# Fleming-Sung/mpc-limX-control

Measured on AMD Instinct MI355X. Metric: QP solves/sec, 13-state N=10 SRBM MPC, batch=65536 at 1/2/4/8 MI355X, higher is better.
Workload: dtype f64; 1 GPU; TRON1 SRBM MPC 13x6 N=10 (box, R = 1e-05 I), linearise+discretise+condense+solve + min-cost selection, global batch 65536 split over 1 GPU(s); global_batch=65536, batch_per_gpu=65536, horizon=10, nx=13, nu=6, config=B, parallelism=dp1, selection=record fused into the solve kernels (last workgroup) (single GPU), max_solver_iters=7, select=fused, kernel=k_mpc_pair, lib_build_id=cfb06c8e6fa2

## Files before the change

include/mpcqp.h:

```cpp
#ifndef MPCQP_H
#define MPCQP_H

#include <stddef.h>
#include <stdint.h>

#ifdef __cplusplus
extern "C" {
#endif

#define MPCQP_OK 0
#define MPCQP_ERR_BAD_DIMS 1
#define MPCQP_ERR_INFEASIBLE 2
#define MPCQP_ERR_ITER_LIMIT 3
#define MPCQP_ERR_NOT_PD 4
#define MPCQP_ERR_DEVICE 5
#define MPCQP_ERR_BAD_ARG 6
#define MPCQP_ERR_NO_DEVICE 7

#define MPCQP_INFTY 1e20

#define MPCQP_MAX_NX 32
#define MPCQP_MAX_NU 16
#define MPCQP_MAX_N 32
#define MPCQP_MAX_NV 256
// ... 132 lines not shown
                    const double *eeVel, const unsigned char *contact, const double *quat,
                    const double *acc);

int mpcqp_enable_timing(mpcqp_ctx *ctx, int on);
double mpcqp_last_kernel_ms(mpcqp_ctx *ctx, int which);
double mpcqp_kernel_ms_sum(mpcqp_ctx *ctx, int which, int *count);

int mpcqp_count_solver_flops(mpcqp_ctx *ctx, int on);
double mpcqp_solver_flops(mpcqp_ctx *ctx, int *launches);

int mpcqp_ctx_pair_dedup(const mpcqp_ctx *ctx);
int mpcqp_ctx_pair_w4_min(const mpcqp_ctx *ctx);
int mpcqp_count_covered(mpcqp_ctx *ctx, int on);
long long mpcqp_covered(mpcqp_ctx *ctx, int *launches);

int mpcqp_debug_phase_cycles(mpcqp_ctx *ctx, uint64_t *out, int n);

const char *mpcqp_status_string(int status);
const char *mpcqp_build_id(void);
int mpcqp_device_count(void);

#ifdef __cplusplus
}
#endif
#endif
```

mpc-limx-control_amd/csrc/fast_kernels.hpp:

```cpp
#pragma once
#include <hip/hip_runtime.h>

#include "../../include/mpcqp.h"

#ifdef MPCQP_VARIANT_TAG
extern "C" const char *mpcqp_variant_tag_fn(void) { return MPCQP_VARIANT_TAG; }
#endif

#ifndef MPCQP_W32
#define MPCQP_W32 3
#endif
#ifndef MPCQP_W64
#define MPCQP_W64 2
#endif
#include "condense.hpp"
#include "fused.hpp"
#include "mpc_fused.hpp"

namespace mpcqp {

struct FastKernels {
    const void *mpc_gen = nullptr;
    const void *pair = nullptr, *pair_gen = nullptr;
    const void *pair_w4 = nullptr, *pair_gen_w4 = nullptr;
    int pair_w4_min = 0;
    int pair_can_dedup = 0;
    int pair_dedup = 0;
    size_t pair_lds = 0;
    const void *wg = nullptr;
    size_t wg_lds = 0;
    int wg_threads = 0;
    const void *dense = nullptr;
    size_t dense_lds = 0;
    int dense_threads = 0;
    const void *disc = nullptr, *cs = nullptr, *mpc = nullptr;
    const void *mpc_list = nullptr;
    size_t disc_lds = 0, cs_lds = 0, mpc_lds = 0;
    int nx = 0, nu = 0;
    int prim_nf = 0;
    int nf = 0;
    int crash_k = 0, crash_p = 0;
    int crash_k_wg = 0, crash_p_wg = 0;
// ... 94 lines not shown
```

mpc-limx-control_amd/csrc/fast_pair.hip:

```cpp
#include <hip/hip_runtime.h>

#include "../../include/mpcqp.h"
#include "fast_kernels.hpp"
#include "mpc_pair.hpp"

namespace mpcqp {
namespace {

template <int NU, int N, int MODEL, bool GEN, int W>
__global__ void __launch_bounds__(64, W) k_mpc_pair(MpcArgs a) {
    extern __shared__ __attribute__((aligned(16))) unsigned char smem_p[];
    pair_mpc<NU, N, MODEL, GEN, W>(a, smem_p);
}

template <int NU, int N, int MODEL>
void add_pair(FastKernels &k) {
    k.pair = (const void *)&k_mpc_pair<NU, N, MODEL, false, 3>;
    k.pair_w4 = (const void *)&k_mpc_pair<NU, N, MODEL, false, 4>;
    if constexpr (MODEL == 0) {
        k.pair_gen = (const void *)&k_mpc_pair<NU, N, MODEL, true, 3>;
        k.pair_gen_w4 = (const void *)&k_mpc_pair<NU, N, MODEL, true, 4>;
    }
    k.pair_lds = PairLayout<NU, N, MODEL>::lds_bytes;
#ifdef MPCQP_INPUT_ALIAS
    k.pair_can_dedup = 0;
#else
    k.pair_can_dedup = (MPCQP_PAIR_SORT && MODEL == 0 && 2 * N <= 32) ? 1 : 0;
#endif
    k.crash_k = MPCQP_PAIR_CRASH ? kPairCrashK : 0;
    k.crash_p = MPCQP_PAIR_CRASH ? kPairCrashP : 0;
}

}

bool add_fast_pair(int model, int N, bool fric, int nfmax, FastKernels &k) {
    static_assert(kPairNF == kPairCap, "one capacity");
    (void)nfmax;
    if (fric || N != 10) return false;
    if (model == MPCQP_MODEL_SRBM && k.nu == 6) { add_pair<6, 10, 0>(k); return true; }
    if (model == MPCQP_MODEL_LITERAL && k.nu == 3) { add_pair<3, 10, 1>(k); return true; }
    return false;
}

// ... 2 lines not shown
```

mpc-limx-control_amd/csrc/mpc_fused.hpp:

```cpp
#pragma once
#include "condense.hpp"
#include "gi_reg.hpp"
#include "gi_solver.hpp"

namespace mpcqp {

#ifndef MPCQP_REG_TILES
#define MPCQP_REG_TILES 1
#endif
template <int NF>
constexpr bool kRegTiles = MPCQP_REG_TILES && NF > 32;

struct MpcArgs {
    int B;
    double Ts, mass;
    double Ibinv[9];
    const double *qd, *pd;
    const double *qm, *pm;
    const double *fq, *fp;
    const double *rmat;
    double fz_min, fz_max, fxy_max, u_min, u_max, mu;
    int max_iter, max_free;
    int crash_p;
    int crash_p_wg;
    double blo_v, blo_t, bhi_v, bhi_t, tlo_v, tlo_t, thi_v, thi_t;
    const double *lin, *x0, *xref;
    const uint64_t *contact;
    double *U, *cost;
    int *status, *iters;
    unsigned long long *stamps;
    double *flops_acc;
    int dedup;
    unsigned long long *cov_acc;
    int cut;
    const double *state;
    const double *feet;
    const double *cmd;
    const double *phase;
    int cands;
    float swing, stance;
    int *ovf;
    int ovf_cap;
    unsigned long long *warm;
    int warm_words;
    unsigned long long *sel;
    long long sel_base;
    long long *sel_rec;
    int sel_final;
// ... 91 lines not shown
    __threadfence();
    sel_final_reduce(a, nV, scratch, tid, kSelNone);
}
__device__ __forceinline__ void sel_commit(const MpcArgs &a, unsigned long long k, int nV,
                                           bool wrote, unsigned long long *scratch, int groups = -1,
                                           bool fresh = false) {
    sel_commit_t(a, k, nV, wrote, scratch, groups, (int)threadIdx.x, fresh);
}

constexpr int kListSubs = 64, kListStride = 32;
constexpr int kListHeadWords = kListSubs * kListStride;
__host__ __device__ constexpr int ovf_list_cap(long long B) {
    return (int)((B + kListSubs - 1) / kListSubs) + 2;
}
__device__ __forceinline__ void wg_list_append(int *list, int cap, int b0, bool d0, int b1,
                                               bool d1) {
    const int n = (d0 ? 1 : 0) + (d1 ? 1 : 0);
    if (!n) return;
    const int s = (int)(blockIdx.x % kListSubs);
    const int i = __hip_atomic_fetch_add(&list[s * kListStride], n, __ATOMIC_RELAXED,
                                         __HIP_MEMORY_SCOPE_AGENT);
    int *ids = list + kListHeadWords + s * cap + i;
    if (d0) *ids++ = b0;
    if (d1) *ids = b1;
}
struct OvfView {
    int *list;
    int cap, cnt, incl, total;
    __device__ __forceinline__ int id(int i) const {
        const int s = __popcll(__ballot(incl <= i));
        const int excl = __shfl(incl - cnt, s, kWave);
        return list[kListHeadWords + s * cap + (i - excl)];
    }
};
// ... 294 lines not shown
    C.L.rowfix = D + Lay::oMisc;
    C.L.ys = D + Lay::oMisc;
    int *ip = reinterpret_cast<int *>(D + Lay::nDoubles);
    C.L.fid = ip;
    C.L.pos = ip + NF;
    C.L.st = reinterpret_cast<unsigned char *>(ip + NF + NV);
    C.L.cb = D + Lay::oCB;

    double lin[8];
    mpc_load_inputs<Lay, NU, N, GEN>(a, b, D, lin);
    MPCQP_CUT(a.cut, 11);
    gi_setup(C);
    if (C.nf > a.max_free || (listed && C.nf > NF)) C.status = ST_BAD_DIMS;
    wave_sync();
    if (!listed && a.ovf && C.nf > NF && C.nf <= a.max_free) {
        if (ln == 0) wg_list_append(a.ovf, a.ovf_cap, b, true, 0, false);
        return;
    }
    mpc_model_terms<Lay, NU, MODEL>(a, D, lin);
    MPCQP_CUT(a.cut, 13);
    MPCQP_STAMP(a.stamps, 0, tst);
    MPCQP_CUT(a.cut, 1);

    mpc_condensed_terms<Lay, NU, N, MODEL>(a, D);
    MPCQP_STAMP(a.stamps, 1, tst);
    MPCQP_CUT(a.cut, 2);

    const int nf = C.nf;
    const bool ok = C.status == ST_OK && nf > 0;
    double gp = 0.0;
    if (ok && ln < nf) {
// ... 87 lines not shown
```

mpc-limx-control_amd/csrc/mpc_pair.hpp:

```cpp
#pragma once
#include "half_ops.hpp"
#include "mpc_fused.hpp"

namespace mpcqp {

template <int W>
constexpr int pair_pf() {
#ifdef MPCQP_PF_DUAL
    return MPCQP_PF_DUAL;
#else
    return W >= 4 ? 4 : 8;
#endif
}
#ifndef MPCQP_PAIR_SORT
#define MPCQP_PAIR_SORT 1
#endif
#ifndef MPCQP_CHOL_CB
#define MPCQP_CHOL_CB 2
#endif
#ifndef MPCQP_CHOL_PF
#define MPCQP_CHOL_PF 4
#endif
#ifndef MPCQP_PAIR_FOLD
#define MPCQP_PAIR_FOLD 1
// ... 96 lines not shown
    const uint64_t right = half_ballot(hl < N && ph < sw);
    const uint64_t left = half_ballot(hl < N && !(ph < sw));
    return spread_even(left) | (spread_even(right) << 1);
}

__device__ __forceinline__ int row_bcast_u32(int v, int j) {
    switch (j) {
#define MPCQP_RB(i) case i: return __builtin_amdgcn_mov_dpp(v, 0x150 + i, 0xf, 0xf, false);
        MPCQP_RB(0) MPCQP_RB(1) MPCQP_RB(2) MPCQP_RB(3) MPCQP_RB(4) MPCQP_RB(5) MPCQP_RB(6)
        MPCQP_RB(7) MPCQP_RB(8) MPCQP_RB(9) MPCQP_RB(10) MPCQP_RB(11) MPCQP_RB(12) MPCQP_RB(13)
        MPCQP_RB(14) MPCQP_RB(15)
#undef MPCQP_RB
        default: return 0;
    }
}
template <bool GEN, int N>
__device__ __forceinline__ int pair_sorted_instance(const MpcArgs &a, unsigned &same,
                                                    unsigned &cand) {
    const int ln = lane(), c = ln & 15;
    int g0, wq;
    if constexpr (!GEN && 2 * N <= 32) {
        const int w = (int)blockIdx.x, ngf = a.B >> 4;
        if (w < 8 * ngf) {
            wq = w / ngf;
            g0 = 16 * (w - wq * ngf);
        } else {
            wq = w - 8 * ngf;
            g0 = 16 * ngf;
        }
    } else {
        const int wv = xcd_order((int)blockIdx.x, (int)gridDim.x);
        g0 = (2 * wv) & ~15;
        wq = wv & 7;
    }
    const int gn = a.B - g0 < 16 ? a.B - g0 : 16;
    int rank = 0;
    [[maybe_unused]] unsigned eq = 0, xw = 0;
    if constexpr (!GEN && 2 * N <= 32) {
        unsigned key = ~0u;
        if (c < gn) key = (unsigned)a.contact[g0 + c];
        if (a.dedup && c < gn) {
            const long long xb = __double_as_longlong(a.x0[(size_t)(g0 + c) * 13 + 3]);
            xw = (unsigned)xb ^ (unsigned)(xb >> 32);
        }
        unsigned lt = 0;
#pragma unroll
        for (int j = 0; j < 16; ++j) {
            const unsigned kj = (unsigned)row_bcast_u32((int)key, j);
            lt |= (j < gn && kj < key) ? (1u << j) : 0u;
            eq |= (j < gn && kj == key) ? (1u << j) : 0u;
        }
        const unsigned below = (1u << c) - 1u;
        const bool first = (eq & below) == 0u;
        const unsigned lead = (unsigned)(__ballot(ln < 16 && c < gn && first) & 0xffffull);
        rank = first ? __popc(lead & lt)
                     : __popc(lead) + __popc(lt & ~lead) + __popc(eq & below) - 1;
    } else {
        unsigned long long key = ~0ull;
// ... 114 lines not shown
    static_assert(!GEN || MODEL == 0, "generated inputs are defined for the SRBM model");
    static_assert(MODEL == 0 || MODEL == 1, "TRON1 models only");
    using Lay = PairLayout<NU, N, MODEL>;
    using Sup = XSupport<MODEL>;
    constexpr int NX = 13, NS = NX + NU, NF = kPairNF, NV = Lay::NV, SD = Lay::SD, NP = kHalf;
#ifdef MPCQP_INPUT_ALIAS
    constexpr bool kDedup = false;
#else
    constexpr bool kDedup = MPCQP_PAIR_SORT && MODEL == 0 && !GEN && 2 * N <= 32;
#endif
    MPCQP_STAMP_INIT(tst);
    const int ln = lane(), hl = ln & (kHalf - 1);
    const bool up = ln >= kHalf;
    int bq = 2 * xcd_order((int)blockIdx.x, (int)gridDim.x) + (up ? 1 : 0);
    unsigned same = 0, cand = 0;
    if constexpr (MPCQP_PAIR_SORT && MODEL == 0) bq = pair_sorted_instance<GEN, N>(a, same, cand);
    bool valid = bq < a.B;
    unsigned cov = 0;
    const int b = valid ? bq : a.B - 1;
    [[maybe_unused]] const int b_ = b;
    unsigned char *Dbase = smem + (up ? Lay::bytes : 0);
    double *D = reinterpret_cast<double *>(Dbase);
    signed char *fid = reinterpret_cast<signed char *>(Dbase + Lay::oFid);
    signed char *pos = reinterpret_cast<signed char *>(Dbase + Lay::oPos);
    double *X0 = D + Lay::oX0, *X1 = D + Lay::oX1, *Ax = D + Lay::oAx, *A2x = D + Lay::oA2x;
    double *xr = D + Lay::oXr, *x0g = D + Lay::oX0v, *UV = D + Lay::oUV;
    double *S = D + Lay::oS;
    const double *Rm = a.rmat;
    const double *Qd = a.qd, *Pd = a.pd;

    double lin[8];
// ... 74 lines not shown
#pragma unroll
                    for (int c = 0; c < NC; ++c)
                        if (half_ballot(d[c] != 0ull) == 0u) cov |= bit[c];
                };
                do {
                    const unsigned tw = (unsigned)__builtin_amdgcn_readlane((int)todo, 0),
                                   tu = (unsigned)__builtin_amdgcn_readlane((int)todo, kHalf);
                    if (((tw & (tw - 1u)) | (tu & (tu - 1u))) == 0u) trip(PairInt<1>{});
                    else trip(PairInt<CH>{});
                } while (__ballot(todo != 0u) != 0ull);
                if (3 * __popcll(contact & kSched) > NF) cov = 0u;
            }
            if (!leads && cov) {
                valid = false;
                cov = 0u;
            }
            if (__ballot(valid) == 0ull) {
                if (a.sel)
                    sel_commit_t(a, kSelNone, NV, false,
                                 reinterpret_cast<unsigned long long *>(smem) + Lay::oR, -1, ln);
                return;
            }
        }
#pragma unroll
        for (int r = 0; r < RX; ++r)
            if (hl + r * kHalf < NXR) xr[hl + r * kHalf] = v[r];
        if (hl < NX) x0g[hl] = x0l;
    }
    wave_sync();
    MPCQP_CUT(a.cut, 11);
// ... 986 lines not shown
    MPCQP_STAMP(a.stamps, 8, tst);
    MPCQP_CUT(a.cut, 7);
    int lno = lane();
    asm volatile("" : "+v"(lno));
    const int hlo = lno & (kHalf - 1);
    double *Do = reinterpret_cast<double *>(smem + (lno >= kHalf ? Lay::bytes : 0));
    const unsigned char *Dob = smem + (lno >= kHalf ? Lay::bytes : 0);
    const signed char *fido = reinterpret_cast<const signed char *>(Dob + Lay::oFid);
    const signed char *poso = reinterpret_cast<const signed char *>(Dob + Lay::oPos);
    const uint64_t *ctlo = reinterpret_cast<const uint64_t *>(Dob + Lay::oCt);
    const int bo = (int)(long long)ctlo[1];
    const bool defer = a.ovf && nf > NF && nf <= a.max_free;
    {
        const int b0 = __builtin_amdgcn_readlane(bo, 0), b1 = __builtin_amdgcn_readlane(bo, kHalf);
        const uint64_t dm = __ballot(defer && bo >= 0);
        if (dm && lno == 0) wg_list_append(a.ovf, a.ovf_cap, b0, dm & 1ull, b1, (dm >> kHalf) & 1ull);
    }
    if constexpr (GEN) {
        if (a.warm) {
            unsigned long long *wl = reinterpret_cast<unsigned long long *>(Do + Lay::oRow);
            wave_sync();
            if (hlo < a.warm_words) wl[hlo] = 0ull;
            wave_sync();
            if (bo >= 0 && hlo < nf && nf <= NF && act2) {
                const int v = fido[hlo];
                if (act2 & 1) atomicOr(&wl[v >> 6], 1ull << (v & 63));
                if (act2 & 2) atomicOr(&wl[(NV + v) >> 6], 1ull << ((NV + v) & 63));
            }
            wave_sync();
            if (bo >= 0 && hlo < a.warm_words) a.warm[(size_t)bo * a.warm_words + hlo] = wl[hlo];
            wave_sync();
// ... 65 lines not shown
```

mpc-limx-control_amd/csrc/mpcqp_kernels.hip:

```cpp
#include <hip/hip_runtime.h>
#include <unistd.h>

#include <math.h>
#include <stdio.h>
#include <stdlib.h>
#include <string.h>

#include <algorithm>
#include <new>
#include <vector>

#include "../../include/mpcqp.h"

#include "fast_kernels.hpp"
#include "gi_solver.hpp"
#include "gi_wg.hpp"

using namespace mpcqp;

namespace {

struct CondenseArgs {
    ModelConst mc;
    int B;
// ... 367 lines not shown
    if (model == MPCQP_MODEL_SRBM && nu == 6) {
        if (N == 10) found = pick_fast_srbm10(fric, nprim, k);
        if (N == 20) found = pick_fast_srbm20(fric, nprim, k);
    }
    if (model == MPCQP_MODEL_LITERAL && nu == 3 && !fric) found = pick_fast_literal(N, nprim, k);
    if (found && pair_enabled()) add_fast_pair(model, N, fric, nprim, k);
    if (k.pair && k.crash_k > 0)
        if (const char *e = getenv("MPCQP_CRASH_P")) k.crash_p = std::max(0, atoi(e));
    if (k.pair) {
        const char *e = getenv("MPCQP_PAIR_DEDUP");
        k.pair_dedup = k.pair_can_dedup && !(e && e[0] == '0');
    }
    if (k.pair) {
        k.pair_w4_min = kPairW4Min;
        if (const char *e = getenv("MPCQP_PAIR_W4_MIN")) k.pair_w4_min = std::max(0, atoi(e));
    }
    if (k.pair)
        if (const char *e = getenv("MPCQP_PAIR_LDS_PAD")) k.pair_lds += (size_t)std::max(0, atoi(e));
    if (found) {
        k.prim_nf = k.pair ? kPairCap : k.nf;
        if (nfmax > k.prim_nf) add_fast_wg(model, N, fric, k);
    }
    if (k.crash_k_wg > 0)
        if (const char *e = getenv("MPCQP_CRASH_P_WG")) k.crash_p_wg = std::max(0, atoi(e));
    return found;
}

void inv3(const double *A, double *Ai) {
    const double a = A[0], b = A[3], c = A[6], d = A[1], e = A[4], f = A[7], g = A[2],
                 h = A[5], i = A[8];
// ... 66 lines not shown
    double *scratchH = nullptr, *scratchF = nullptr;
    size_t scratch_cap = 0;
    bool fast = false;
    FastKernels fk;
    double *dqd = nullptr, *dpd = nullptr;
    double *dFQ = nullptr, *dFP = nullptr;
    double *dAB = nullptr;
    size_t ab_cap = 0;
    unsigned long long *dstamps = nullptr;
    double *dflops = nullptr;
    bool flops_on = false;
    int flops_launches = 0;
    unsigned long long *dcov = nullptr;
    bool cov_on = false;
    int cov_launches = 0;
    unsigned long long *dsel = nullptr;
    int *dlist = nullptr;
    size_t list_cap = 0;
    int list_par = 0;
    int wg_grid = 0;
    void *hbuf = nullptr;
    size_t hbuf_cap = 0;
    void *pin = nullptr;
    size_t pin_cap = 0;
    hipStream_t hstream = nullptr;
    hipEvent_t hev = nullptr;
    hipStream_t hs_in = nullptr, hs_out = nullptr;
    hipEvent_t hev_in[8] = {}, hev_k[8] = {};
    bool hd_ok = false;
    bool hd_off = false;
// ... 372 lines not shown
                     hipMemcpy(c->dFQ, fq.data(), sizeof(double) * nx * nx, hipMemcpyHostToDevice) != hipSuccess ||
                     hipMemcpy(c->dFP, fp.data(), sizeof(double) * nx * nx, hipMemcpyHostToDevice) != hipSuccess)) {
            mpcqp_ctx_destroy(c);
            return MPCQP_ERR_DEVICE;
        }
        if (pick_fast_dense(nx, nu, m->N, toep, c->fk)) {
            c->fast = true;
            set_lds(c->fk.dense, c->fk.dense_lds);
            if (const char *e = getenv("MPCQP_CRASH_P_WG")) c->fk.crash_p_wg = std::max(0, atoi(e));
        }
    }
    if (!c->fast && nfmax > kWave) {
        mpcqp_ctx_destroy(c);
        return MPCQP_ERR_BAD_DIMS;
    }
    if (c->fast && c->fk.wg) {
        int dev_cus = 0, nb = 0;
        hipDeviceGetAttribute(&dev_cus, hipDeviceAttributeMultiprocessorCount, device);
        set_lds(c->fk.wg, c->fk.wg_lds);
        hipOccupancyMaxActiveBlocksPerMultiprocessor(&nb, c->fk.wg, c->fk.wg_threads, c->fk.wg_lds);
        c->wg_grid = std::max(1, nb) * std::max(1, dev_cus);
    }
    c->m.Q = c->m.R = c->m.P = nullptr;
    *out = c;
    return MPCQP_OK;
}

int mpcqp_ctx_fast_path(const mpcqp_ctx *c) {
    if (!c || !c->fast) return 0;
    if (c->fk.dense) return 3;
// ... 47 lines not shown
        hipStreamSynchronize(c->stream) != hipSuccess)
        return -1.0;
    for (int i = 0; i < kFlopsSlots; ++i) v += h[i * kFlopsStride];
    if (launches) *launches = c->flops_launches;
    c->flops_launches = 0;
    return v;
}

int mpcqp_ctx_pair_dedup(const mpcqp_ctx *c) {
    return c && c->fast && c->fk.pair && !c->fk.dense ? c->fk.pair_dedup : 0;
}

int mpcqp_ctx_pair_w4_min(const mpcqp_ctx *c) {
    if (!c || !c->fast || !c->fk.pair || c->fk.dense || !c->fk.pair_w4) return 0;
    return c->fk.pair_w4_min;
}

int mpcqp_count_covered(mpcqp_ctx *c, int on) {
    if (!c) return MPCQP_ERR_BAD_ARG;
    if (on && !c->dcov) {
        hipSetDevice(c->device);
        if (hipMalloc(&c->dcov, sizeof(unsigned long long) * kFlopsWords) != hipSuccess ||
            hipMemsetAsync(c->dcov, 0, sizeof(unsigned long long) * kFlopsWords, c->stream) != hipSuccess) {
            hipFree(c->dcov);
            c->dcov = nullptr;
            return MPCQP_ERR_DEVICE;
        }
    }
    c->cov_on = on != 0;
    return MPCQP_OK;
// ... 41 lines not shown
int mpcqp_ctx_destroy(mpcqp_ctx *c) {
    if (!c) return MPCQP_ERR_BAD_ARG;
    hipSetDevice(c->device);
    if (c->stream) hipStreamSynchronize(c->stream);
    hipFree(c->dQ);
    hipFree(c->dR);
    hipFree(c->dP);
    hipFree(c->dqd);
    hipFree(c->dpd);
    hipFree(c->dFQ);
    hipFree(c->dFP);
    hipFree(c->dAB);
    hipFree(c->dstamps);
    hipFree(c->dflops);
    hipFree(c->dcov);
    hipFree(c->dsel);
    hipFree(c->dlist);
    hipFree(c->hbuf);
    for (int i = 0; i < 3; ++i)
        if (c->hg_exec[i]) hipGraphExecDestroy(c->hg_exec[i]);
    if (c->pin) hipHostFree(c->pin);
    if (c->hev) hipEventDestroy(c->hev);
    if (c->hstream) hipStreamDestroy(c->hstream);
    for (int i = 0; i < 8; ++i) {
        if (c->hev_in[i]) hipEventDestroy(c->hev_in[i]);
        if (c->hev_k[i]) hipEventDestroy(c->hev_k[i]);
    }
    if (c->hs_in) hipStreamDestroy(c->hs_in);
    if (c->hs_out) hipStreamDestroy(c->hs_out);
    hipFree(c->rbuf);
// ... 11 lines not shown
}

int mpcqp_set_stream(mpcqp_ctx *c, void *stream) {
    if (!c) return MPCQP_ERR_BAD_ARG;
    if (c->own_stream && c->stream) {
        hipStreamSynchronize(c->stream);
        hipStreamDestroy(c->stream);
    }
    c->own_stream = false;
    c->stream = (hipStream_t)stream;
    return MPCQP_OK;
}

int mpcqp_sync(mpcqp_ctx *c) {
    if (!c) return MPCQP_ERR_BAD_ARG;
    return hip_status(hipStreamSynchronize(c->stream));
}

int mpcqp_enable_timing(mpcqp_ctx *c, int on) {
    if (!c) return MPCQP_ERR_BAD_ARG;
    if (on && !c->ev_ok) {
        hipSetDevice(c->device);
        hipEvent_t *evs = &c->ev[0][0][0];
        constexpr int nev = 4 * mpcqp_ctx::kTimingRing * 2;
        for (int i = 0; i < nev; ++i)
            if (hipEventCreate(&evs[i]) != hipSuccess) {
                for (int j = 0; j < i; ++j) hipEventDestroy(evs[j]);
                return MPCQP_ERR_DEVICE;
            }
        c->ev_ok = true;
    }
// ... 107 lines not shown
    {
        const bool lit = m.model == MPCQP_MODEL_LITERAL;
        a.blo_v = lit ? m.u_min : m.fz_min;
        a.blo_t = lit ? m.u_min : -m.fxy_max;
        a.bhi_v = lit ? -m.u_max : -m.fz_max;
        a.bhi_t = lit ? -m.u_max : -m.fxy_max;
        a.tlo_v = -kFeasTol * (1.0 + fabs(a.blo_v));
        a.tlo_t = -kFeasTol * (1.0 + fabs(a.blo_t));
        a.thi_v = -kFeasTol * (1.0 + fabs(a.bhi_v));
        a.thi_t = -kFeasTol * (1.0 + fabs(a.bhi_t));
    }
    a.stamps = c->dstamps;
    a.flops_acc = c->flops_on ? c->dflops : nullptr;
    a.dedup = c->fk.pair_dedup;
    a.cov_acc = c->cov_on ? c->dcov : nullptr;
    a.cut = 0;
#ifdef MPCQP_CUTS
    if (const char *e = getenv("MPCQP_CUT")) a.cut = atoi(e);
#endif
    return a;
}

static int launch(const void *k, int B, size_t lds, hipStream_t s, void *arg) {
    void *args[] = {arg};
    return hip_status(hipLaunchKernel(k, dim3(B), dim3(64), args, lds, s));
}

static int ensure_bytes(mpcqp_ctx *c, void **buf, size_t *cap, size_t bytes) {
    if (*cap >= bytes) return MPCQP_OK;
    if (*buf) hipStreamSynchronize(c->stream);
// ... 42 lines not shown
    if (c->dlist) hipStreamSynchronize(c->stream);
    hipFree(c->dlist);
    c->dlist = nullptr;
    c->list_cap = 0;
    ++c->buf_gen;
    const size_t stride = list_stride((size_t)B);
    if (hipMalloc(&c->dlist, sizeof(int) * 2 * stride) != hipSuccess ||
        hipMemsetAsync(c->dlist, 0, sizeof(int) * kListHeadWords, c->stream) != hipSuccess ||
        hipMemsetAsync(c->dlist + stride, 0, sizeof(int) * kListHeadWords, c->stream) != hipSuccess)
        return MPCQP_ERR_DEVICE;
    c->list_cap = B;
    c->list_par = 0;
    return MPCQP_OK;
}

static int launch_mpc(mpcqp_ctx *c, bool gen, int B, MpcArgs *a, bool may_overflow = true) {
    a->ovf = nullptr;
    int *list = nullptr, *rearm = nullptr;
    if (c->fk.wg && !gen && may_overflow) {
        const int rc = ensure_list(c, B);
        if (rc) return rc;
        const size_t stride = list_stride(c->list_cap);
        list = c->dlist + (c->list_par ? stride : 0);
        rearm = c->dlist + (c->list_par ? 0 : stride);
        a->ovf = list;
        a->ovf_cap = ovf_list_cap((long long)c->list_cap);
    }
    const void *pk = gen ? c->fk.pair_gen : c->fk.pair;
    if (pk && B >= c->fk.pair_w4_min && c->fk.pair_w4_min > 0) {
        const void *p4 = gen ? c->fk.pair_gen_w4 : c->fk.pair_w4;
        if (p4) pk = p4;
    }
    a->sel_final = a->ovf ? 0 : 1;
    if (a->flops_acc && pk) ++c->flops_launches;
    if (a->cov_acc && pk) ++c->cov_launches;
    tbegin(c, 2);
    int rc = pk ? launch(pk, (B + 1) / 2, c->fk.pair_lds, c->stream, a)
                : launch(gen ? c->fk.mpc_gen : c->fk.mpc, B, c->fk.mpc_lds, c->stream, a);
    tend(c, 2);
    if (rc || !a->ovf) return rc;
    a->sel_final = 1;
    void *args[] = {a, &list, &rearm};
    const int grid = std::max(1, std::min(B, c->wg_grid));
    tbegin(c, 3);
    rc = hip_status(hipLaunchKernel(c->fk.wg, dim3(grid), dim3(c->fk.wg_threads), args, c->fk.wg_lds,
                                    c->stream));
    tend(c, 3);
    c->list_par ^= 1;
    return rc;
}

int mpcqp_batch_condense(mpcqp_ctx *c, int B, const double *x0, const double *xref,
                         const double *lin, double *H, double *f) {
    if (!c || !x0 || !xref || !lin || !H || !f || B < 0) return MPCQP_ERR_BAD_ARG;
    if (B == 0) return MPCQP_OK;
    hipSetDevice(c->device);
    CondenseArgs a = batch_condense_args(c, B, x0, xref, lin, H, f);
    const size_t lds = set_lds((const void *)k_condense,
                               sizeof(double) * condense_lds_doubles(c->m.nx, c->m.nu, c->m.N));
    tbegin(c, 0);
    hipLaunchKernelGGL(k_condense, dim3(B), dim3(64), lds, c->stream, a);
    tend(c, 0);
    return hip_status(hipGetLastError());
// ... 205 lines not shown
        return rc;
    }
    int rc = mpcqp_batch_solve(c, B, x0, xref, lin, contact, U, cost, status, iters);
    if (!rc) rc = mpcqp_batch_select_record(c, B, cost, status, U, index_base, record);
    return rc;
}

int mpcqp_ctx_reserve(mpcqp_ctx *c, int B) {
    if (!c || B < 0) return MPCQP_ERR_BAD_ARG;
    if (B == 0) return MPCQP_OK;
    hipSetDevice(c->device);
    const size_t ab = (size_t)c->m.nx * (c->m.nx + c->m.nu);
    int rc = ensure_bytes(c, &c->hbuf, &c->hbuf_cap, host_stage_bytes(c, B));
    if (!rc) rc = ensure_bytes(c, &c->fkbuf, &c->fkbuf_cap, sizeof(double) * 15 * (size_t)B);
    if (!rc && c->fast && c->fk.wg) rc = ensure_list(c, B);
    if (!rc && c->fast && c->fk.mpc_gen)
        rc = ensure_bytes(c, &c->rbuf, &c->rbuf_cap, rollout_bytes(c, B, 1));
    if (!rc && c->warm_on && c->fast && c->fk.mpc_gen) rc = ensure_warm(c, B);
    if (!rc && !c->fast) rc = ensure_bytes(c, (void **)&c->dAB, &c->ab_cap, sizeof(double) * ab * B);
    if (!rc && !c->fast) rc = ensure_scratch_hf(c, B);
    if (!rc) rc = hip_status(hipStreamSynchronize(c->stream));
    return rc;
}

int mpcqp_ctx_fk_feet_host(mpcqp_ctx *c, int R, const double *q, const double *rpy,
                           int rpy_stride, double *feet) {
    if (!c || !q || !rpy || !feet || R < 0 || rpy_stride < 3) return MPCQP_ERR_BAD_ARG;
    if (R == 0) return MPCQP_OK;
    hipSetDevice(c->device);
    const size_t nq = 6 * (size_t)R, nr = (size_t)rpy_stride * (R - 1) + 3, nf = 6 * (size_t)R;
// ... 165 lines not shown
    const size_t b_x0 = sizeof(double) * nx * B, b_xr = sizeof(double) * nx * (N + 1) * B,
                 b_lin = sizeof(double) * lin_w * B, b_ct = contact ? sizeof(uint64_t) * B : 0;
    const size_t in_bytes = b_x0 + b_xr + b_lin + sizeof(uint64_t) * B;
    const size_t out_off = (in_bytes + 15) & ~(size_t)15;
    const size_t b_u = sizeof(double) * nV * B, b_c = sizeof(double) * B, b_i = sizeof(int) * B;
    const size_t out_bytes = b_u + b_c + 2 * b_i, total = out_off + out_bytes;
    if (ensure_bytes(c, &c->hbuf, &c->hbuf_cap, std::max(total, host_stage_bytes(c, B))))
        return MPCQP_ERR_DEVICE;
    if (!c->hstream) {
        if (hipStreamCreateWithFlags(&c->hstream, hipStreamNonBlocking) != hipSuccess ||
            hipEventCreateWithFlags(&c->hev, hipEventDisableTiming) != hipSuccess)
            return MPCQP_ERR_DEVICE;
    }
    const bool ovf = host_may_overflow(c, B, contact);
    if (ovf && ensure_list(c, B)) return MPCQP_ERR_DEVICE;
    if (B >= kHostDirectMin && !c->hd_off && host_locked(x0, b_x0) && host_locked(xref, b_xr) &&
        host_locked(lin, b_lin) && (!contact || host_locked(contact, b_ct)) &&
        host_locked(U, b_u) && host_locked(cost, b_c) && host_locked(status, b_i) &&
        host_locked(iters, b_i)) {
        if (hipEventRecord(c->hev, c->stream) != hipSuccess) return MPCQP_ERR_DEVICE;
        return host_direct(c, B, x0, xref, lin, contact, U, cost, status, iters, ovf, out_off);
    }
    if (c->pin_cap < total) {
        if (c->pin) hipHostFree(c->pin);
        c->pin = nullptr;
        c->pin_cap = 0;
        ++c->buf_gen;
        if (hipHostMalloc(&c->pin, total, hipHostMallocDefault) != hipSuccess) return MPCQP_ERR_DEVICE;
        c->pin_cap = total;
    }
// ... 212 lines not shown
```

mpc-limx-control_amd/mpcqp/_lib.py:

```python
from __future__ import annotations

import ctypes as C
import os

_PKG = os.path.dirname(os.path.abspath(__file__))
LIB_PATH = os.environ.get("MPCQP_LIB") or os.path.join(os.path.dirname(_PKG), "lib",
                                                       "libmpcqp.so")

MPCQP_OK = 0
STATUS = {0: "OK", 1: "BAD_DIMS", 2: "INFEASIBLE", 3: "ITER_LIMIT", 4: "NOT_PD", 5: "DEVICE",
          6: "BAD_ARG", 7: "NO_DEVICE"}
MPCQP_INFTY = 1e20
MODEL_SRBM, MODEL_LITERAL, MODEL_DENSE = 0, 1, 2
CONS_BOX, CONS_FRICTION = 0, 1
A_ROWMAJOR, A_COLMAJOR = 0, 1

EXPORTS = [
    "mpcqp_discretize", "mpcqp_discretize_quadrature", "mpcqp_build_qp", "mpcqp_solve_dense", "mpcqp_plant_step",
    "mpcqp_ctx_create", "mpcqp_ctx_destroy", "mpcqp_set_stream", "mpcqp_sync",
    "mpcqp_batch_condense", "mpcqp_batch_solve_qp", "mpcqp_batch_solve",
    "mpcqp_ctx_fast_path", "mpcqp_ctx_one_wave_nf", "mpcqp_ctx_overflow_kernel", "mpcqp_ctx_crash_params", "mpcqp_batch_discretize", "mpcqp_batch_condense_solve",
    "mpcqp_debug_phase_cycles", "mpcqp_batch_solve_host",
    "mpcqp_count_solver_flops", "mpcqp_solver_flops",
    "mpcqp_ctx_pair_dedup", "mpcqp_ctx_pair_w4_min", "mpcqp_count_covered", "mpcqp_covered",
    "mpcqp_batch_select_min", "mpcqp_batch_select_record", "mpcqp_reduce_records",
    "mpcqp_batch_solve_select",
    "mpcqp_enable_timing", "mpcqp_last_kernel_ms", "mpcqp_kernel_ms_sum",
    "mpcqp_batch_solve_gait", "mpcqp_batch_select_state", "mpcqp_batch_plant_srbm",
    "mpcqp_rollout", "mpcqp_fk_feet", "mpcqp_kf_update", "mpcqp_ctx_reserve",
    "mpcqp_ctx_fk_feet_host", "mpcqp_set_warm_start",
    "mpcqp_shard", "mpcqp_group_create", "mpcqp_group_unique_id", "mpcqp_group_create_rank",
    "mpcqp_group_destroy", "mpcqp_group_info", "mpcqp_group_ctx", "mpcqp_group_solve_select",
    "mpcqp_group_wait", "mpcqp_group_sync", "mpcqp_group_solve_select_host",
    "mpcqp_group_wait_stream", "mpcqp_group_failed",
    "mpcqp_host_register", "mpcqp_host_unregister", "mpcqp_host_alloc", "mpcqp_host_free",
    "mpcqp_status_string", "mpcqp_device_count", "mpcqp_build_id",
]


# ... 41 lines not shown
    for name, at in (("mpcqp_ctx_one_wave_nf", [vp]), ("mpcqp_ctx_crash_params", [vp] + [vp] * 4),
                     ("mpcqp_ctx_overflow_kernel", [vp])):
        if hasattr(L, name):
            getattr(L, name).argtypes = at
    L.mpcqp_debug_phase_cycles.argtypes = [vp, vp, i]
    if hasattr(L, "mpcqp_count_solver_flops"):
        L.mpcqp_count_solver_flops.argtypes = [vp, i]
        L.mpcqp_solver_flops.argtypes = [vp, C.POINTER(C.c_int)]
        L.mpcqp_solver_flops.restype = C.c_double
    if hasattr(L, "mpcqp_count_covered"):
        L.mpcqp_ctx_pair_dedup.argtypes = [vp]
        L.mpcqp_ctx_pair_w4_min.argtypes = [vp]
        L.mpcqp_count_covered.argtypes = [vp, i]
        L.mpcqp_covered.argtypes = [vp, C.POINTER(C.c_int)]
        L.mpcqp_covered.restype = C.c_longlong
    L.mpcqp_batch_solve_host.argtypes = [vp, i] + [vp] * 8
    L.mpcqp_batch_discretize.argtypes = [vp, i, vp, vp]
    L.mpcqp_batch_condense_solve.argtypes = [vp, i] + [vp] * 8
    L.mpcqp_batch_select_min.argtypes = [vp, i, vp, vp, C.c_int64, vp]
    L.mpcqp_batch_select_record.argtypes = [vp, i, vp, vp, vp, C.c_int64, vp]
    L.mpcqp_reduce_records.argtypes = [vp, i, vp, vp]
    if hasattr(L, "mpcqp_batch_solve_select"):
        L.mpcqp_batch_solve_select.argtypes = [vp, i] + [vp] * 8 + [C.c_int64, vp]
    L.mpcqp_batch_solve_gait.argtypes = [vp, i, i] + [vp] * 4 + [C.c_float, C.c_float] + [vp] * 4
    L.mpcqp_batch_select_state.argtypes = [vp, i, i] + [vp] * 6
    L.mpcqp_batch_plant_srbm.argtypes = [vp, i, i] + [vp] * 5
    L.mpcqp_rollout.argtypes = [vp, i, i, i] + [vp] * 4 + [C.c_float, C.c_float, vp, vp]
    L.mpcqp_fk_feet.argtypes = [vp, i, vp, vp, i, vp]
    L.mpcqp_ctx_fk_feet_host.argtypes = [vp, i, vp, vp, i, vp]
    L.mpcqp_ctx_reserve.argtypes = [vp, i]
# ... 41 lines not shown
```

mpc-limx-control_amd/mpcqp/engine.py:

```python
from __future__ import annotations

import ctypes as C

import numpy as np

from . import model as _model
from ._lib import check, lib


def _ptr(t):
    return C.c_void_p(t.data_ptr()) if t is not None else None


class BatchEngine:

    def __init__(self, params: dict, device: int = 0, stream=None):
        import torch

        self.torch = torch
        self.p = params
        self.device = device
        self.nV = params["nu"] * params["N"]
        m, keep = _model.to_struct(params)
        ctx = C.c_void_p()
# ... 199 lines not shown
    def pair_dedup(self) -> bool:
        return bool(lib().mpcqp_ctx_pair_dedup(self.ctx))

    @property
    def pair_w4_min(self) -> int:
        return int(lib().mpcqp_ctx_pair_w4_min(self.ctx))

    def count_covered(self, on=True):
        check("mpcqp_count_covered", lib().mpcqp_count_covered(self.ctx, 1 if on else 0))

    def covered(self):
        n = C.c_int(0)
        v = int(lib().mpcqp_covered(self.ctx, C.byref(n)))
        return v, n.value

    def last_kernel_ms(self, which: int) -> float:
        return float(lib().mpcqp_last_kernel_ms(self.ctx, which))

    def kernel_ms_sum(self, which: int):
        n = C.c_int(0)
        ms = float(lib().mpcqp_kernel_ms_sum(self.ctx, which, C.byref(n)))
        return ms, n.value


def decode_key(key: int):
    idx = key & 0x7FFFFFFF
    ob = (key >> 31) & 0xFFFFFFFF
    bits = (ob & 0x7FFFFFFF) if (ob & 0x80000000) else (~ob & 0xFFFFFFFF)
    cost = np.frombuffer(np.uint32(bits).tobytes(), dtype=np.float32)[0]
    return float(cost), int(idx)
# ... 7 lines not shown
```

Before: 559.6 million QP/s.

## Add cross-wavefront hint words so deduplicated pair groups skip redundant waves

Adds a per-16-instance-group counter word in device memory. The wave with wq==0 records whether its deduplicated solve already covered every instance in the group; later waves for the same group check the word and exit early, committing an empty selection record. An optional mode also splits the pair launch into four ordered sub-launches so leader waves are scheduled first. This is meant to cut redundant wavefront work when duplicate instances are common, at the cost of extra atomics, host-side occupancy queries and buffer resets. Skip behaviour depends on scheduling order, so the benefit may vary between runs.

```diff
diff --git a/include/mpcqp.h b/include/mpcqp.h
--- a/include/mpcqp.h
+++ b/include/mpcqp.h
@@ -170,6 +170,10 @@
 int mpcqp_count_covered(mpcqp_ctx *ctx, int on);
 long long mpcqp_covered(mpcqp_ctx *ctx, int *launches);
 
+int mpcqp_ctx_pair_hint(const mpcqp_ctx *ctx, int *min_wavefronts, int *min_wavefronts_w4);
+int mpcqp_count_skipped(mpcqp_ctx *ctx, int on);
+long long mpcqp_skipped(mpcqp_ctx *ctx, int *launches);
+
 int mpcqp_debug_phase_cycles(mpcqp_ctx *ctx, uint64_t *out, int n);
 
 const char *mpcqp_status_string(int status);
diff --git a/mpc-limx-control_amd/csrc/fast_kernels.hpp b/mpc-limx-control_amd/csrc/fast_kernels.hpp
--- a/mpc-limx-control_amd/csrc/fast_kernels.hpp
+++ b/mpc-limx-control_amd/csrc/fast_kernels.hpp
@@ -26,6 +26,8 @@
     int pair_w4_min = 0;
     int pair_can_dedup = 0;
     int pair_dedup = 0;
+    int pair_can_hint = 0, pair_hint = 0, pair_cap = 0, pair_cap_w4 = 0;
+    int pair_hint_rounds = 4;
     size_t pair_lds = 0;
     const void *wg = nullptr;
     size_t wg_lds = 0;
diff --git a/mpc-limx-control_amd/csrc/fast_pair.hip b/mpc-limx-control_amd/csrc/fast_pair.hip
--- a/mpc-limx-control_amd/csrc/fast_pair.hip
+++ b/mpc-limx-control_amd/csrc/fast_pair.hip
@@ -27,6 +27,7 @@
 #else
     k.pair_can_dedup = (MPCQP_PAIR_SORT && MODEL == 0 && 2 * N <= 32) ? 1 : 0;
 #endif
+    k.pair_can_hint = k.pair_can_dedup;
     k.crash_k = MPCQP_PAIR_CRASH ? kPairCrashK : 0;
     k.crash_p = MPCQP_PAIR_CRASH ? kPairCrashP : 0;
 }
diff --git a/mpc-limx-control_amd/csrc/mpc_fused.hpp b/mpc-limx-control_amd/csrc/mpc_fused.hpp
--- a/mpc-limx-control_amd/csrc/mpc_fused.hpp
+++ b/mpc-limx-control_amd/csrc/mpc_fused.hpp
@@ -32,6 +32,9 @@
     double *flops_acc;
     int dedup;
     unsigned long long *cov_acc;
+    unsigned *hint;
+    unsigned long long *skip_acc;
+    int item0;
     int cut;
     const double *state;
     const double *feet;
@@ -153,10 +156,10 @@
     return (int)((B + kListSubs - 1) / kListSubs) + 2;
 }
 __device__ __forceinline__ void wg_list_append(int *list, int cap, int b0, bool d0, int b1,
-                                               bool d1) {
+                                               bool d1, unsigned w) {
     const int n = (d0 ? 1 : 0) + (d1 ? 1 : 0);
     if (!n) return;
-    const int s = (int)(blockIdx.x % kListSubs);
+    const int s = (int)(w % kListSubs);
     const int i = __hip_atomic_fetch_add(&list[s * kListStride], n, __ATOMIC_RELAXED,
                                          __HIP_MEMORY_SCOPE_AGENT);
     int *ids = list + kListHeadWords + s * cap + i;
@@ -481,7 +484,7 @@
     if (C.nf > a.max_free || (listed && C.nf > NF)) C.status = ST_BAD_DIMS;
     wave_sync();
     if (!listed && a.ovf && C.nf > NF && C.nf <= a.max_free) {
-        if (ln == 0) wg_list_append(a.ovf, a.ovf_cap, b, true, 0, false);
+        if (ln == 0) wg_list_append(a.ovf, a.ovf_cap, b, true, 0, false, blockIdx.x);
         return;
     }
     mpc_model_terms<Lay, NU, MODEL>(a, D, lin);
diff --git a/mpc-limx-control_amd/csrc/mpc_pair.hpp b/mpc-limx-control_amd/csrc/mpc_pair.hpp
--- a/mpc-limx-control_amd/csrc/mpc_pair.hpp
+++ b/mpc-limx-control_amd/csrc/mpc_pair.hpp
@@ -134,13 +134,22 @@
         default: return 0;
     }
 }
+constexpr unsigned kHintDone = 0x100u, kHintCount = 0xffu;
+__device__ __forceinline__ bool hint_arrive(unsigned *word, unsigned add, unsigned ng) {
+    const unsigned old = __hip_atomic_fetch_add(word, add, __ATOMIC_RELAXED, __HIP_MEMORY_SCOPE_AGENT);
+    if ((old & kHintCount) + 1u == ng)
+        __hip_atomic_store(word, 0u, __ATOMIC_RELAXED, __HIP_MEMORY_SCOPE_AGENT);
+    return (old & kHintDone) != 0u;
+}
+
 template <bool GEN, int N>
 __device__ __forceinline__ int pair_sorted_instance(const MpcArgs &a, unsigned &same,
-                                                    unsigned &cand) {
+                                                    unsigned &cand, int &it_g0, int &it_wq,
+                                                    bool &done) {
     const int ln = lane(), c = ln & 15;
     int g0, wq;
     if constexpr (!GEN && 2 * N <= 32) {
-        const int w = (int)blockIdx.x, ngf = a.B >> 4;
+        const int w = (int)blockIdx.x + a.item0, ngf = a.B >> 4;
         if (w < 8 * ngf) {
             wq = w / ngf;
             g0 = 16 * (w - wq * ngf);
@@ -154,6 +163,9 @@
         wq = wv & 7;
     }
     const int gn = a.B - g0 < 16 ? a.B - g0 : 16;
+    it_g0 = g0;
+    it_wq = wq;
+    done = false;
     int rank = 0;
     [[maybe_unused]] unsigned eq = 0, xw = 0;
     if constexpr (!GEN && 2 * N <= 32) {
@@ -162,6 +174,15 @@
         if (a.dedup && c < gn) {
             const long long xb = __double_as_longlong(a.x0[(size_t)(g0 + c) * 13 + 3]);
             xw = (unsigned)xb ^ (unsigned)(xb >> 32);
+        }
+        if (a.hint && wq > 0) {
+            bool d = false;
+            if (ln == 0) d = hint_arrive(a.hint + (g0 >> 4), 1u, (unsigned)((gn + 1) >> 1));
+            if (__ballot(d) != 0ull) {
+                done = true;
+                same = cand = 0;
+                return a.B;
+            }
         }
         unsigned lt = 0;
 #pragma unroll
@@ -306,7 +327,21 @@
     const bool up = ln >= kHalf;
     int bq = 2 * xcd_order((int)blockIdx.x, (int)gridDim.x) + (up ? 1 : 0);
     unsigned same = 0, cand = 0;
-    if constexpr (MPCQP_PAIR_SORT && MODEL == 0) bq = pair_sorted_instance<GEN, N>(a, same, cand);
+    [[maybe_unused]] int it_g0 = 0, it_wq = 0;
+    if constexpr (MPCQP_PAIR_SORT && MODEL == 0) {
+        bool done = false;
+        bq = pair_sorted_instance<GEN, N>(a, same, cand, it_g0, it_wq, done);
+        if constexpr (kDedup) {
+            if (done) {
+                if (a.skip_acc && ln == 0)
+                    atomicAdd(a.skip_acc + (blockIdx.x % kFlopsSlots) * kFlopsStride, 1ull);
+                if (a.sel)
+                    sel_commit_t(a, kSelNone, NV, false,
+                                 reinterpret_cast<unsigned long long *>(smem) + Lay::oR, -1, ln);
+                return;
+            }
+        }
+    }
     bool valid = bq < a.B;
     unsigned cov = 0;
     const int b = valid ? bq : a.B - 1;
@@ -411,6 +446,14 @@
             if (!leads && cov) {
                 valid = false;
                 cov = 0u;
+            }
+            if (a.hint && it_wq == 0) {
+                const int gn = a.B - it_g0 < 16 ? a.B - it_g0 : 16;
+                const int acc = valid ? 1 + __popc(cov) : 0;
+                const bool all =
+                    __builtin_amdgcn_readlane(acc, 0) + __builtin_amdgcn_readlane(acc, kHalf) == gn;
+                if (gn > 2 && ln == 0)
+                    hint_arrive(a.hint + (it_g0 >> 4), all ? kHintDone + 1u : 1u, (unsigned)((gn + 1) >> 1));
             }
             if (__ballot(valid) == 0ull) {
                 if (a.sel)
@@ -1427,7 +1470,9 @@
     {
         const int b0 = __builtin_amdgcn_readlane(bo, 0), b1 = __builtin_amdgcn_readlane(bo, kHalf);
         const uint64_t dm = __ballot(defer && bo >= 0);
-        if (dm && lno == 0) wg_list_append(a.ovf, a.ovf_cap, b0, dm & 1ull, b1, (dm >> kHalf) & 1ull);
+        if (dm && lno == 0)
+            wg_list_append(a.ovf, a.ovf_cap, b0, dm & 1ull, b1, (dm >> kHalf) & 1ull,
+                           blockIdx.x + (kDedup ? (unsigned)a.item0 : 0u));
     }
     if constexpr (GEN) {
         if (a.warm) {
diff --git a/mpc-limx-control_amd/csrc/mpcqp_kernels.hip b/mpc-limx-control_amd/csrc/mpcqp_kernels.hip
--- a/mpc-limx-control_amd/csrc/mpcqp_kernels.hip
+++ b/mpc-limx-control_amd/csrc/mpcqp_kernels.hip
@@ -405,6 +405,12 @@
     if (k.pair) {
         k.pair_w4_min = kPairW4Min;
         if (const char *e = getenv("MPCQP_PAIR_W4_MIN")) k.pair_w4_min = std::max(0, atoi(e));
+    }
+    if (k.pair) {
+        const char *e = getenv("MPCQP_PAIR_HINT");
+        k.pair_hint = !(k.pair_can_hint && k.pair_dedup) || (e && e[0] == '0') ? 0
+                      : (e && (e[0] == '2' || e[0] == '3')) ? e[0] - '0' : 1;
+        if (const char *r = getenv("MPCQP_PAIR_HINT_ROUNDS")) k.pair_hint_rounds = std::max(0, atoi(r));
     }
     if (k.pair)
         if (const char *e = getenv("MPCQP_PAIR_LDS_PAD")) k.pair_lds += (size_t)std::max(0, atoi(e));
@@ -501,6 +507,12 @@
     unsigned long long *dcov = nullptr;
     bool cov_on = false;
     int cov_launches = 0;
+    unsigned *dpair = nullptr;
+    size_t pair_groups = 0;
+    bool pair_dirty = false;
+    unsigned long long *dskip = nullptr;
+    bool skip_on = false;
+    int skip_launches = 0;
     unsigned long long *dsel = nullptr;
     int *dlist = nullptr;
     size_t list_cap = 0;
@@ -903,6 +915,25 @@
         mpcqp_ctx_destroy(c);
         return MPCQP_ERR_BAD_DIMS;
     }
+    if (c->fast && c->fk.pair && c->fk.pair_hint) {
+        int dev_cus = 0, nb = 0, nb4 = 0;
+        bool ok = hipDeviceGetAttribute(&dev_cus, hipDeviceAttributeMultiprocessorCount, device) == hipSuccess &&
+                  dev_cus > 0;
+        set_lds(c->fk.pair, c->fk.pair_lds);
+        ok = ok && hipOccupancyMaxActiveBlocksPerMultiprocessor(&nb, c->fk.pair, 64, c->fk.pair_lds) == hipSuccess &&
+             nb > 0;
+        if (ok && c->fk.pair_w4) {
+            set_lds(c->fk.pair_w4, c->fk.pair_lds);
+            ok = hipOccupancyMaxActiveBlocksPerMultiprocessor(&nb4, c->fk.pair_w4, 64, c->fk.pair_lds) == hipSuccess &&
+                 nb4 > 0;
+        }
+        if (ok) {
+            c->fk.pair_cap = nb * dev_cus;
+            c->fk.pair_cap_w4 = c->fk.pair_w4 ? nb4 * dev_cus : c->fk.pair_cap;
+        } else {
+            c->fk.pair_hint = 0;
+        }
+    }
     if (c->fast && c->fk.wg) {
         int dev_cus = 0, nb = 0;
         hipDeviceGetAttribute(&dev_cus, hipDeviceAttributeMultiprocessorCount, device);
@@ -980,6 +1011,45 @@
 int mpcqp_ctx_pair_w4_min(const mpcqp_ctx *c) {
     if (!c || !c->fast || !c->fk.pair || c->fk.dense || !c->fk.pair_w4) return 0;
     return c->fk.pair_w4_min;
+}
+
+int mpcqp_ctx_pair_hint(const mpcqp_ctx *c, int *min_wavefronts, int *min_wavefronts_w4) {
+    const bool on = c && c->fast && c->fk.pair && !c->fk.dense && c->fk.pair_hint;
+    if (min_wavefronts)
+        *min_wavefronts = !on ? 0 : c->fk.pair_hint >= 2 ? 1 : c->fk.pair_hint_rounds * c->fk.pair_cap + 1;
+    if (min_wavefronts_w4)
+        *min_wavefronts_w4 = !on ? 0 : c->fk.pair_hint >= 2 ? 1 : c->fk.pair_hint_rounds * c->fk.pair_cap_w4 + 1;
+    return on ? 1 : 0;
+}
+
+int mpcqp_count_skipped(mpcqp_ctx *c, int on) {
+    if (!c) return MPCQP_ERR_BAD_ARG;
+    if (on && !c->dskip) {
+        hipSetDevice(c->device);
+        if (hipMalloc(&c->dskip, sizeof(unsigned long long) * kFlopsWords) != hipSuccess ||
+            hipMemsetAsync(c->dskip, 0, sizeof(unsigned long long) * kFlopsWords, c->stream) != hipSuccess) {
+            hipFree(c->dskip);
+            c->dskip = nullptr;
+            return MPCQP_ERR_DEVICE;
+        }
+    }
+    c->skip_on = on != 0;
+    return MPCQP_OK;
+}
+
+long long mpcqp_skipped(mpcqp_ctx *c, int *launches) {
+    if (launches) *launches = 0;
+    if (!c || !c->dskip) return -1;
+    unsigned long long h[kFlopsWords], v = 0;
+    hipSetDevice(c->device);
+    if (hipMemcpyAsync(h, c->dskip, sizeof h, hipMemcpyDeviceToHost, c->stream) != hipSuccess ||
+        hipMemsetAsync(c->dskip, 0, sizeof h, c->stream) != hipSuccess ||
+        hipStreamSynchronize(c->stream) != hipSuccess)
+        return -1;
+    for (int i = 0; i < kFlopsSlots; ++i) v += h[i * kFlopsStride];
+    if (launches) *launches = c->skip_launches;
+    c->skip_launches = 0;
+    return (long long)v;
 }
 
 int mpcqp_count_covered(mpcqp_ctx *c, int on) {
@@ -1051,6 +1121,8 @@
     hipFree(c->dstamps);
     hipFree(c->dflops);
     hipFree(c->dcov);
+    hipFree(c->dpair);
+    hipFree(c->dskip);
     hipFree(c->dsel);
     hipFree(c->dlist);
     hipFree(c->hbuf);
@@ -1092,7 +1164,9 @@
 
 int mpcqp_sync(mpcqp_ctx *c) {
     if (!c) return MPCQP_ERR_BAD_ARG;
-    return hip_status(hipStreamSynchronize(c->stream));
+    const int rc = hip_status(hipStreamSynchronize(c->stream));
+    if (rc) c->pair_dirty = true;
+    return rc;
 }
 
 int mpcqp_enable_timing(mpcqp_ctx *c, int on) {
@@ -1230,6 +1304,7 @@
     a.flops_acc = c->flops_on ? c->dflops : nullptr;
     a.dedup = c->fk.pair_dedup;
     a.cov_acc = c->cov_on ? c->dcov : nullptr;
+    a.skip_acc = c->skip_on ? c->dskip : nullptr;
     a.cut = 0;
 #ifdef MPCQP_CUTS
     if (const char *e = getenv("MPCQP_CUT")) a.cut = atoi(e);
@@ -1302,6 +1377,32 @@
     return MPCQP_OK;
 }
 
+static int ensure_pair(mpcqp_ctx *c, int B) {
+    const size_t groups = ((size_t)B + 15) / 16;
+    if (c->dpair && c->pair_groups >= groups) {
+        if (!c->pair_dirty) return MPCQP_OK;
+        int rc = hip_status(hipStreamSynchronize(c->stream));
+        if (!rc) rc = hip_status(hipMemsetAsync(c->dpair, 0, sizeof(unsigned) * c->pair_groups, c->stream));
+        if (!rc) c->pair_dirty = false;
+        return rc;
+    }
+    c->pair_dirty = false;
+    if (c->dpair) hipStreamSynchronize(c->stream);
+    hipFree(c->dpair);
+    c->dpair = nullptr;
+    c->pair_groups = 0;
+    ++c->buf_gen;
+    const size_t bytes = sizeof(unsigned) * groups;
+    if (hipMalloc(&c->dpair, bytes) != hipSuccess ||
+        hipMemsetAsync(c->dpair, 0, bytes, c->stream) != hipSuccess)
+        return MPCQP_ERR_DEVICE;
+    c->pair_groups = groups;
+    return MPCQP_OK;
+}
+static bool pair_hints(const mpcqp_ctx *c, bool gen) {
+    return !gen && c->fast && c->fk.pair && c->fk.pair_hint;
+}
+
 static int launch_mpc(mpcqp_ctx *c, bool gen, int B, MpcArgs *a, bool may_overflow = true) {
     a->ovf = nullptr;
     int *list = nullptr, *rearm = nullptr;
@@ -1315,17 +1416,45 @@
         a->ovf_cap = ovf_list_cap((long long)c->list_cap);
     }
     const void *pk = gen ? c->fk.pair_gen : c->fk.pair;
+    bool w4 = false;
     if (pk && B >= c->fk.pair_w4_min && c->fk.pair_w4_min > 0) {
         const void *p4 = gen ? c->fk.pair_gen_w4 : c->fk.pair_w4;
-        if (p4) pk = p4;
-    }
+        if (p4) {
+            pk = p4;
+            w4 = true;
+        }
+    }
+    a->hint = nullptr;
+    a->item0 = 0;
+    if (pk && pair_hints(c, gen)) {
+        const int cap = w4 ? c->fk.pair_cap_w4 : c->fk.pair_cap;
+        if (c->fk.pair_hint >= 2 || (long long)(B + 1) / 2 > (long long)c->fk.pair_hint_rounds * cap) {
+            const int rc = ensure_pair(c, B);
+            if (rc) return rc;
+            a->hint = c->dpair;
+        }
+    }
+    if (a->skip_acc && pk) ++c->skip_launches;
     a->sel_final = a->ovf ? 0 : 1;
     if (a->flops_acc && pk) ++c->flops_launches;
     if (a->cov_acc && pk) ++c->cov_launches;
     tbegin(c, 2);
-    int rc = pk ? launch(pk, (B + 1) / 2, c->fk.pair_lds, c->stream, a)
+    int rc = MPCQP_OK;
+    if (pk && a->hint && c->fk.pair_hint == 3 && !a->sel) {
+        const int items = (B + 1) / 2, ngf = B >> 4, r[4][2] = {{0, ngf}, {8 * ngf, std::min(items, 8 * ngf + 1)},
+                                                                 {ngf, 8 * ngf}, {8 * ngf + 1, items}};
+        for (int i = 0; i < 4 && !rc; ++i) {
+            if (r[i][1] <= r[i][0]) continue;
+            a->item0 = r[i][0];
+            rc = launch(pk, r[i][1] - r[i][0], c->fk.pair_lds, c->stream, a);
+        }
+        a->item0 = 0;
+    } else {
+        rc = pk ? launch(pk, (B + 1) / 2, c->fk.pair_lds, c->stream, a)
                 : launch(gen ? c->fk.mpc_gen : c->fk.mpc, B, c->fk.mpc_lds, c->stream, a);
+    }
     tend(c, 2);
+    if (rc) c->pair_dirty = true;
     if (rc || !a->ovf) return rc;
     a->sel_final = 1;
     void *args[] = {a, &list, &rearm};
@@ -1335,6 +1464,7 @@
                                     c->stream));
     tend(c, 3);
     c->list_par ^= 1;
+    if (rc) c->pair_dirty = true;
     return rc;
 }
 
@@ -1570,6 +1700,7 @@
     int rc = ensure_bytes(c, &c->hbuf, &c->hbuf_cap, host_stage_bytes(c, B));
     if (!rc) rc = ensure_bytes(c, &c->fkbuf, &c->fkbuf_cap, sizeof(double) * 15 * (size_t)B);
     if (!rc && c->fast && c->fk.wg) rc = ensure_list(c, B);
+    if (!rc && pair_hints(c, false)) rc = ensure_pair(c, B);
     if (!rc && c->fast && c->fk.mpc_gen)
         rc = ensure_bytes(c, &c->rbuf, &c->rbuf_cap, rollout_bytes(c, B, 1));
     if (!rc && c->warm_on && c->fast && c->fk.mpc_gen) rc = ensure_warm(c, B);
@@ -1765,6 +1896,7 @@
     }
     const bool ovf = host_may_overflow(c, B, contact);
     if (ovf && ensure_list(c, B)) return MPCQP_ERR_DEVICE;
+    if (pair_hints(c, false) && ensure_pair(c, B)) return MPCQP_ERR_DEVICE;
     if (B >= kHostDirectMin && !c->hd_off && host_locked(x0, b_x0) && host_locked(xref, b_xr) &&
         host_locked(lin, b_lin) && (!contact || host_locked(contact, b_ct)) &&
         host_locked(U, b_u) && host_locked(cost, b_c) && host_locked(status, b_i) &&
diff --git a/mpc-limx-control_amd/mpcqp/_lib.py b/mpc-limx-control_amd/mpcqp/_lib.py
--- a/mpc-limx-control_amd/mpcqp/_lib.py
+++ b/mpc-limx-control_amd/mpcqp/_lib.py
@@ -23,6 +23,7 @@
     "mpcqp_debug_phase_cycles", "mpcqp_batch_solve_host",
     "mpcqp_count_solver_flops", "mpcqp_solver_flops",
     "mpcqp_ctx_pair_dedup", "mpcqp_ctx_pair_w4_min", "mpcqp_count_covered", "mpcqp_covered",
+    "mpcqp_ctx_pair_hint", "mpcqp_count_skipped", "mpcqp_skipped",
     "mpcqp_batch_select_min", "mpcqp_batch_select_record", "mpcqp_reduce_records",
     "mpcqp_batch_solve_select",
     "mpcqp_enable_timing", "mpcqp_last_kernel_ms", "mpcqp_kernel_ms_sum",
@@ -94,6 +95,11 @@
         L.mpcqp_count_covered.argtypes = [vp, i]
         L.mpcqp_covered.argtypes = [vp, C.POINTER(C.c_int)]
         L.mpcqp_covered.restype = C.c_longlong
+    if hasattr(L, "mpcqp_count_skipped"):
+        L.mpcqp_ctx_pair_hint.argtypes = [vp, C.POINTER(C.c_int), C.POINTER(C.c_int)]
+        L.mpcqp_count_skipped.argtypes = [vp, i]
+        L.mpcqp_skipped.argtypes = [vp, C.POINTER(C.c_int)]
+        L.mpcqp_skipped.restype = C.c_longlong
     L.mpcqp_batch_solve_host.argtypes = [vp, i] + [vp] * 8
     L.mpcqp_batch_discretize.argtypes = [vp, i, vp, vp]
     L.mpcqp_batch_condense_solve.argtypes = [vp, i] + [vp] * 8
diff --git a/mpc-limx-control_amd/mpcqp/engine.py b/mpc-limx-control_amd/mpcqp/engine.py
--- a/mpc-limx-control_amd/mpcqp/engine.py
+++ b/mpc-limx-control_amd/mpcqp/engine.py
@@ -237,6 +237,20 @@
         v = int(lib().mpcqp_covered(self.ctx, C.byref(n)))
         return v, n.value
 
+    @property
+    def pair_hint(self) -> tuple:
+        n3, n4 = C.c_int(0), C.c_int(0)
+        on = bool(lib().mpcqp_ctx_pair_hint(self.ctx, C.byref(n3), C.byref(n4)))
+        return on, n3.value, n4.value
+
+    def count_skipped(self, on=True):
+        check("mpcqp_count_skipped", lib().mpcqp_count_skipped(self.ctx, 1 if on else 0))
+
+    def skipped(self):
+        n = C.c_int(0)
+        v = int(lib().mpcqp_skipped(self.ctx, C.byref(n)))
+        return v, n.value
+
     def last_kernel_ms(self, which: int) -> float:
         return float(lib().mpcqp_last_kernel_ms(self.ctx, which))
 
```

Result: faster. 581.5 million QP/s (median of 6 runs) (+3.9%).
